# HydrogenSulfate/LFT

Measured on AMD Instinct MI355X. Metric: LF patches/sec (5x5 angRes, 32x32 LR, 4xSR), higher is better.
Workload: dtype bf16; 1 GPU; LFT 5x5 angRes 4xSR inference, batch=4 per GPU, 32x32 LR patches; global_batch=4, parallelism=dp1 (independent shards), streams_per_gpu=1, hip_graph=True, steps_in_flight=2

## Files before the change

### lft_amd/csrc/lft_api.hip

```cpp
#include "../../include/lft_hip.h"
#include "../../include/lft_hip_test.h"
#include <hip/hip_runtime.h>
#include <stdint.h>

#include <cstdarg>
#include <cstdio>
#include <cmath>
#include <map>
#include <mutex>
#include <set>
#include <string>
#include <algorithm>
#include <type_traits>
#include <utility>
#include <vector>

#ifndef LFT_TU
#define LFT_TU 0
#endif

namespace {
#include "lft_kernels_a.cuh"
#include "lft_kernels_b.cuh"
#include "lft_metrics.cuh"
// ... 38 lines not shown
    std::vector<const char*> names;
};
thread_local Profiler g_prof;
inline const char* prof_name(const char* plain, const char* fmt, ...) {
    if (!g_prof.on) return plain;
    static thread_local std::set<std::string> names;
    char buf[96];
    va_list ap;
    va_start(ap, fmt);
    vsnprintf(buf, sizeof(buf), fmt, ap);
    va_end(ap);
    return names.insert(buf).first->c_str();
}
inline void prof_mark(const char* name) {
    if (!g_prof.on) return;
    hipEvent_t e;
    if (hipEventCreate(&e) != hipSuccess) return;
    (void)hipEventRecord(e, g_prof.st);
    g_prof.ev.push_back(e);
    g_prof.names.push_back(name);
}

#define LFT_LAUNCH_OK(name)                                                                  \
    do {                                                                                     \
        hipError_t e_ = hipGetLastError();                                                   \
        if (e_ != hipSuccess) return fail((int)e_, "launch %s: %s", name, hipGetErrorString(e_)); \
        prof_mark(name);                                                                     \
    } while (0)
template <typename Run> int run_profiled(hipStream_t st, int max_records, float* ms_out, const char** names_out, int* n_out, Run&& run) {
    g_prof.on = true; g_prof.st = st; g_prof.ev.clear(); g_prof.names.clear();
    prof_mark("start");
    const int rc = run();
    g_prof.on = false;
    hipError_t e = hipStreamSynchronize(st);
    int n = 0;
    for (size_t i = 1; i < g_prof.ev.size() && n < max_records; ++i, ++n) {
        float ms = 0.0f;
        (void)hipEventElapsedTime(&ms, g_prof.ev[i - 1], g_prof.ev[i]);
        ms_out[n] = ms;
        names_out[n] = g_prof.names[i];
    }
    for (hipEvent_t ev : g_prof.ev) (void)hipEventDestroy(ev);
    g_prof.ev.clear(); g_prof.names.clear();
    *n_out = n;
    if (rc) return rc;
    if (e != hipSuccess) return fail((int)e, "hipStreamSynchronize: %s", hipGetErrorString(e));
    return 0;
}

constexpr int kLayers = 4;

template <auto... Vs, typename V, typename F> int dispatch(V v, F&& f) {
    int rc = 0;
    if (((v == Vs && ((rc = f(std::integral_constant<decltype(Vs), Vs>{})), true)) || ...)) return rc;
    return fail(LFT_ERR_ARG, "internal: no kernel variant for %d", (int)v);
}
template <int V> using int_c = std::integral_constant<int, V>;
template <typename F> int by_prec(int prec, F&& f) {
    if (prec == LFT_PREC_F32) return f(float{});
    if (prec == LFT_PREC_BF16) return f(bf16_t{});
    return f(f16_t{});
}
inline size_t align256(size_t x) { return (x + 255) & ~(size_t)255; }

struct Dims {
    int B, A, V, h, w, hw, s, gp, gt, nchunk;
    long long ntok;
};

int make_dims(int B, int A, int h, int w, int s, int prec, Dims* d) {
    if (prec != LFT_PREC_F32 && prec != LFT_PREC_BF16 && prec != LFT_PREC_F16)
        return fail(LFT_ERR_ARG, "prec must be LFT_PREC_F32, LFT_PREC_BF16 or LFT_PREC_F16, got %d", prec);
    if (B < 1 || A < 1 || h < 1 || w < 1) return fail(LFT_ERR_SHAPE, "B, A, h, w must be positive (B=%d A=%d h=%d w=%d)", B, A, h, w);
    if (s != 2 && s != 4) return fail(LFT_ERR_SHAPE, "scale factor must be 2 or 4, got %d", s);
    if (A * A > 128) return fail(LFT_ERR_UNSUPPORTED, "angRes %d (A*A=%d views > 128) is not implemented in this build", A, A * A);
    if ((long long)B * A * A * h * w > (1LL << 27)) return fail(LFT_ERR_SHAPE, "too many tokens");
    d->B = B; d->A = A; d->V = A * A; d->h = h; d->w = w; d->hw = h * w; d->s = s;
    d->gp = (s + 2) * (s + 2); d->gt = (d->gp + 31) / 32; d->nchunk = 2 * s * s;
    d->ntok = (long long)B * d->V * d->hw;
    return 0;
}

constexpr int kFragsConv = 72, kFragsAng = 64, kFragsSpa1 = 240, kFragsSpa1NoQ = 208, kFragsSpa2 = 176;
inline int frags_up(const Dims& d) { return d.nchunk * (4 + 2 * d.gt); }

struct PackedLayout {
    size_t conv0_w, ln_ang[kLayers], ln_spa[kLayers], ang_pe, petok[kLayers], spa_pe_img;
    size_t w01, s_w01;
    size_t s_conv[3], s_ang[kLayers], s_spa1[kLayers], s_spa2[kLayers], s_up, total;
};

PackedLayout packed_layout(const Dims& d, int prec) {
    const size_t esz = prec == LFT_PREC_F32 ? 4 : 2, fragb = 64 * 8 * esz;
    PackedLayout L;
    size_t o = 0;
    auto take = [&](size_t bytes) { size_t r = o; o = align256(o + bytes); return r; };
    L.conv0_w = take(576 * 4);
    for (int l = 0; l < kLayers; ++l) { L.ln_ang[l] = take(256 * 4); L.ln_spa[l] = take(512 * 4); }
    L.ang_pe = take((size_t)((d.V + 31) / 32) * 2048 * 4);
    for (int l = 0; l < kLayers; ++l) L.petok[l] = take((size_t)((d.hw + 32 * kNwSpa1 - 1) / (32 * kNwSpa1)) * kNwSpa1 * 4096 * esz);
    L.spa_pe_img = take((size_t)d.hw * 64 * esz);
    const bool lp = prec != LFT_PREC_F32;
    L.w01 = take(lp ? 64 * kW01K * 4 : 0);
    L.s_conv[0] = take(kFragsConv * fragb);
    L.s_w01 = take(lp ? kW01Frags * fragb : 0);
    for (int i = 1; i < 3; ++i) L.s_conv[i] = take(kFragsConv * fragb);
    for (int l = 0; l < kLayers; ++l) {
        L.s_ang[l] = take(kFragsAng * fragb);
        L.s_spa1[l] = take(kFragsSpa1 * fragb);
        L.s_spa2[l] = take(kFragsSpa2 * fragb);
    }
    L.s_up = take((size_t)frags_up(d) * fragb);
    L.total = o;
    return L;
}

struct WorkLayout {
    size_t x0, feat, xa, xb, tok, q, k, v, o, g, status, total;
};
WorkLayout work_layout(const Dims& d, int prec) {
    const size_t esz = prec == LFT_PREC_F32 ? 4 : 2;
    WorkLayout W;
    size_t o = 0;
    auto take = [&](size_t bytes) { size_t r = o; o = align256(o + bytes); return r; };
    const size_t n = (size_t)d.ntok;
    W.x0 = take(n * 64 * esz); W.feat = take(n * 64 * esz); W.xa = take(n * 64 * esz); W.xb = take(n * 64 * esz);
    W.tok = take(n * 128 * esz); W.q = take(n * 128 * esz); W.k = take(n * 128 * esz); W.v = take(n * 128 * esz);
    W.o = take(n * 128 * esz);
    W.g = take(n * d.gp * 4);
    W.status = take(256);
    W.total = o;
    return W;
}

template <typename T> size_t lds_conv64(int w) { return WRing<T, kConv64Chunk, kNwConv>::LDS_BYTES + ConvIn<T, kNwConv>::bytes(w) + kNwConv * TileIO<2, T>::BYTES + kConvZeroRow; }
template <typename T> size_t lds_conv64_lr(int w) { return lds_conv64<T>(w) + std::max<size_t>(LrStage<kNwConv>::bytes(w), kConv0WBytes); }
constexpr size_t kLdsParams = 1024;
template <typename T, int CH = kSpaChunk> size_t lds_spa1(int w) {
    return WRing<T, CH, kNwSpa1>::LDS_BYTES + std::max<size_t>(ConvIn<T, kNwSpa1>::bytes(w), (size_t)kNwSpa1 * TileIO<4, T>::BYTES) + kLdsParams + kConvZeroRow;
}
template <typename T> size_t lds_spa2() { return WRing<T, kSpaChunk, kNwSpa2>::LDS_BYTES + kLdsParams + kNwSpa2 * TileIO<4, T>::BYTES; }
template <typename T> size_t lds_up() { return WRing<T, kUpChunk, kNwUp>::LDS_BYTES + kNwUp * TileIO<2, T>::BYTES; }
template <typename T> size_t lds_ang() { return (size_t)kFragsAng * 1024 * FragInfo<T>::PIECES + kLdsParams + 4 * TileIO<2, T>::BYTES; }
constexpr size_t kMaxLds = 160 * 1024;
template <typename K> int allow_lds(K kernel, size_t bytes, const char* name) {
    if (bytes > kMaxLds) return fail(LFT_ERR_SHAPE, "%s needs %zu B of LDS (> 160 KiB): view width too large for this build", name, bytes);
    if (bytes <= 64 * 1024) return 0;
    struct Done { int dev; const void* fn; size_t bytes; };
    static thread_local std::vector<Done> done;
    const void* fn = reinterpret_cast<const void*>(kernel);
    int dev = 0;
    LFT_HIP_OK(hipGetDevice(&dev));
    for (const auto& d : done)
        if (d.dev == dev && d.fn == fn && d.bytes >= bytes) return 0;
    LFT_HIP_OK(hipFuncSetAttribute(fn, hipFuncAttributeMaxDynamicSharedMemorySize, (int)bytes));
    done.push_back(Done{dev, fn, bytes});
    return 0;
}

template <typename P> P* at(const void* base, size_t off) { return reinterpret_cast<P*>(const_cast<char*>(static_cast<const char*>(base)) + off); }
inline unsigned blocks_for(long long items, int per_block) { return (unsigned)((items + per_block - 1) / per_block); }

PackOp lin_op(const float* src, int row0, int nrows, int ld, int k0, int ksteps, int kmap, float scale, int kmul = 1, int kadd = 0) {
    PackOp p{};
    p.src = src; p.kind = 0; p.row0 = row0; p.nrows = nrows; p.ntiles = (nrows + 31) / 32; p.ld = ld;
    p.kmul = kmul; p.kadd = kadd; p.k0 = k0; p.ksteps = ksteps; p.kmap = kmap; p.scale = scale; p.s = 0; p.frag0 = 0;
    return p;
}
void conv_ops(std::vector<PackOp>& v, const float* w, int nout) {
    for (int tap = 0; tap < 9; ++tap)
        for (int ks = 0; ks < 4; ++ks) v.push_back(lin_op(w, 0, nout, 576, 16 * ks, 1, 0, 1.0f, 9, tap));
}

template <typename T>
int run_pack(std::vector<PackOp>& ops, T* dst, int expect_frags, hipStream_t st) {
    int total = 0;
    size_t i = 0;
    while (i < ops.size()) {
        PackArgs a{};
        int nf = 0;
        while (i < ops.size() && a.nops < LFT_PACK_MAXOPS) {
            a.op[a.nops] = ops[i];
            a.op[a.nops].frag0 = nf;
            nf += ops[i].ntiles * ops[i].ksteps;
            ++a.nops; ++i;
        }
        k_pack<T><<<nf, 64, 0, st>>>(a, dst + (size_t)total * 512);
        LFT_LAUNCH_OK("k_pack");
        total += nf;
    }
    if (total != expect_frags) return fail(LFT_ERR_ARG, "internal: stream has %d fragments, expected %d", total, expect_frags);
    return 0;
}

template <typename T> bool tok_lane_major(const Dims& d) {
// ... 4 lines not shown
                int nimg, const Dims& d, hipStream_t st, unsigned* status) {
    const size_t l16 = lds_spa1<T, 16>(d.w), l8 = lds_spa1<T, 8>(d.w);
    const size_t share = kMaxLds / kSpaOcc;
    const bool use8 = (l16 > share && l8 <= share) || l16 > kMaxLds;
    const bool lm = !PE_ONLY && tok_lane_major<T>(d);
    return dispatch<8, 16>(use8 ? 8 : 16, [&](auto CH) {
        return dispatch<true, false>(lm, [&](auto LM) {
            constexpr bool WQ = !(LM && sizeof(T) == 2);
            const size_t lds = CH == 8 ? l8 : l16;
            if (int rc = allow_lds(k_spa1<T, PE_ONLY, CH, LM, WQ>, lds, "k_spa1")) return rc;
            k_spa1<T, PE_ONLY, CH, LM, WQ><<<nwg, 64 * kNwSpa1, lds, st>>>(in, ws, ln, petok, tok, q, k, v, pe_out, nimg, d.h, d.w, status);
            return 0;
        });
    });
}

template <typename T>
int pack_impl(const float* const* P, void* packed, const Dims& d, int prec, hipStream_t st) {
    const PackedLayout L = packed_layout(d, prec);
    const float kAngScale = 0.35355339059327373f * LFT_LOG2E;
    const float kSpaScale = 0.25f * LFT_LOG2E;
    int rc;
    k_copy_f32<<<3, 256, 0, st>>>(P[0], at<float>(packed, L.conv0_w), 576);
    LFT_LAUNCH_OK("k_copy_f32");
    for (int i = 0; i < 3; ++i) {
        std::vector<PackOp> ops;
        conv_ops(ops, P[1 + i], 64);
        if ((rc = run_pack<T>(ops, at<T>(packed, L.s_conv[i]), kFragsConv, st))) return rc;
    }
    if constexpr (sizeof(T) == 2) {
        k_compose_w01<<<blocks_for(64 * kW01K, 256), 256, 0, st>>>(P[0], P[1], at<float>(packed, L.w01));
        LFT_LAUNCH_OK("k_compose_w01");
        std::vector<PackOp> ops{lin_op(at<float>(packed, L.w01), 0, 64, kW01K, 0, kW01K / 16, 0, 1.0f)};
        if ((rc = run_pack<ConvLrOp>(ops, at<ConvLrOp>(packed, L.s_w01), kW01Frags, st))) return rc;
    }
    k_pe_tables<T><<<blocks_for(std::max<long long>((long long)((d.V + 31) / 32) * 2048, (long long)d.hw * 64), 256), 256, 0, st>>>(
        at<float>(packed, L.ang_pe), at<T>(packed, L.spa_pe_img), d.V, d.h, d.w);
    LFT_LAUNCH_OK("k_pe_tables");
    for (int l = 0; l < kLayers; ++l) {
        const float* const* q = P + 4 + 18 * l;
        float* lnS = at<float>(packed, L.ln_spa[l]);
        float* lnA = at<float>(packed, L.ln_ang[l]);
        const int srcS[4] = {1, 2, 5, 6}, srcA[4] = {10, 11, 14, 15};
        for (int j = 0; j < 4; ++j) {
            k_copy_f32<<<1, 256, 0, st>>>(q[srcS[j]], lnS + 128 * j, 128);
            k_copy_f32<<<1, 256, 0, st>>>(q[srcA[j]], lnA + 64 * j, 64);
        }
        LFT_LAUNCH_OK("k_copy_f32");
        {
            std::vector<PackOp> ops;
            ops.push_back(lin_op(q[12], 0, 64, 64, 0, 4, 1, kAngScale));
            ops.push_back(lin_op(q[12], 64, 64, 64, 0, 4, 1, 1.0f));
            ops.push_back(lin_op(q[12], 128, 64, 64, 0, 4, 1, 1.0f));
            ops.push_back(lin_op(q[13], 0, 64, 64, 0, 4, 1, 1.0f));
            ops.push_back(lin_op(q[16], 0, 128, 64, 0, 4, 1, 1.0f));
            ops.push_back(lin_op(q[17], 0, 64, 128, 0, 8, 1, 1.0f));
            if ((rc = run_pack<T>(ops, at<T>(packed, L.s_ang[l]), kFragsAng, st))) return rc;
        }
        {
            std::vector<PackOp> ops;
            conv_ops(ops, q[0], 128);
            ops.push_back(lin_op(q[3], 256, 128, 128, 0, 8, 1, 1.0f));
            ops.push_back(lin_op(q[3], 128, 128, 128, 0, 8, 1, 1.0f));
            ops.push_back(lin_op(q[3], 0, 128, 128, 0, 8, 1, kSpaScale));
            if ((rc = run_pack<T>(ops, at<T>(packed, L.s_spa1[l]), kFragsSpa1, st))) return rc;
        }
        {
            std::vector<PackOp> ops;
            ops.push_back(lin_op(q[4], 0, 128, 128, 0, 8, (sizeof(T) == 2 && tok_lane_major<T>(d)) ? 1 : 0, 1.0f));
            for (int c = 0; c < 4; ++c) {
                ops.push_back(lin_op(q[7], 64 * c, 64, 128, 0, 8, 1, 1.0f));
                ops.push_back(lin_op(q[8], 0, 128, 256, 64 * c, 4, 1, 1.0f));
            }
            ops.push_back(lin_op(q[9], 0, 64, 128, 0, 8, 1, 1.0f));
            if ((rc = run_pack<T>(ops, at<T>(packed, L.s_spa2[l]), kFragsSpa2, st))) return rc;
        }
        if ((rc = launch_spa1<T, true>((unsigned)((d.hw + 32 * kNwSpa1 - 1) / (32 * kNwSpa1)), at<T>(packed, L.spa_pe_img), at<T>(packed, L.s_spa1[l]), nullptr, nullptr,
                                       nullptr, nullptr, nullptr, nullptr, at<T>(packed, L.petok[l]), 1, d, st, nullptr))) return rc;
        LFT_LAUNCH_OK("k_spa1<pe>");
    }
    {
        std::vector<PackOp> ops;
        for (int c = 0; c < d.nchunk; ++c) {
            ops.push_back(lin_op(P[76], 32 * c, 32, 64, 0, 4, 1, 1.0f));
            PackOp m = lin_op(P[77], 0, d.gp, 0, 32 * c, 2, 1, 1.0f);
            m.kind = 1; m.s = d.s; m.ntiles = d.gt;
            ops.push_back(m);
        }
        if ((rc = run_pack<T>(ops, at<T>(packed, L.s_up), frags_up(d), st))) return rc;
    }
    return 0;
}

void launch_assemble(const float* lr, const float* g, float* out, int B, int A, int h, int w, int s, hipStream_t st, int gld = 0, unsigned* status = nullptr) {
    const dim3 tg((unsigned)((A * w + 7) / 8) * (unsigned)((A * h + 7) / 8) * (unsigned)B);
    if (!gld) gld = (s + 2) * (s + 2);
    if (s == 2) k_assemble_t<2><<<tg, 256, 0, st>>>(lr, g, out, B, A, h, w, gld, status);
    else k_assemble_t<4><<<tg, 256, 0, st>>>(lr, g, out, B, A, h, w, gld, status);
}

template <typename T>
int init_features_x0(const void* packed, const PackedLayout& L, const float* lr, T* x0, T* ta, T* tb, T* feat, const Dims& d, hipStream_t st) {
    const int nimg = d.B * d.V, nwg = nimg * ((d.hw + 32 * kNwConv - 1) / (32 * kNwConv));
    const size_t lds = lds_conv64<T>(d.w);
    int rc;
    if ((rc = allow_lds(k_conv64<T, 0>, lds, "k_conv64"))) return rc;
    if ((rc = allow_lds(k_conv64<T, 1>, lds, "k_conv64"))) return rc;
    k_conv0<T><<<dim3((unsigned)((d.hw + kConv0Tok - 1) / kConv0Tok), (unsigned)nimg), 256, 0, st>>>(lr, at<float>(packed, L.conv0_w), x0, d.B, d.A, d.h, d.w);
    LFT_LAUNCH_OK("k_conv0");
    k_conv64<T, 0><<<nwg, 64 * kNwConv, lds, st>>>(x0, ta, nullptr, at<T>(packed, L.s_conv[0]), nimg, d.h, d.w, ConvLr{});
    LFT_LAUNCH_OK("k_conv64");
    k_conv64<T, 0><<<nwg, 64 * kNwConv, lds, st>>>(ta, tb, nullptr, at<T>(packed, L.s_conv[1]), nimg, d.h, d.w, ConvLr{});
    LFT_LAUNCH_OK("k_conv64");
    k_conv64<T, 1><<<nwg, 64 * kNwConv, lds, st>>>(tb, feat, x0, at<T>(packed, L.s_conv[2]), nimg, d.h, d.w, ConvLr{});
    LFT_LAUNCH_OK("k_conv64");
    return 0;
}
template <typename T>
int init_features(const void* packed, const PackedLayout& L, const float* lr, T* x0, T* ta, T* tb, T* feat, const Dims& d, hipStream_t st) {
    if constexpr (sizeof(T) == 4) return init_features_x0<T>(packed, L, lr, x0, ta, tb, feat, d, st);
    else {
        const int nimg = d.B * d.V, nwg = nimg * ((d.hw + 32 * kNwConv - 1) / (32 * kNwConv));
        const size_t lds = lds_conv64_lr<T>(d.w);
        int rc;
        if (L.s_w01 + kW01Frags * 1024 != L.s_conv[1]) return fail(LFT_ERR_ARG, "internal: W01 fragments are not in front of conv_init.2's stream");
        if ((rc = allow_lds(k_conv64_lr<T>, lds, "k_conv64"))) return rc;
        if ((rc = allow_lds(k_conv64<T, 2>, lds, "k_conv64"))) return rc;
        k_conv64_lr<T><<<nwg, 64 * kNwConv, lds, st>>>(lr, tb, at<T>(packed, L.s_w01), d.A, nimg, d.h, d.w);
        LFT_LAUNCH_OK("k_conv64");
        k_conv64<T, 2><<<nwg, 64 * kNwConv, lds, st>>>(tb, feat, nullptr, at<T>(packed, L.s_conv[2]), nimg, d.h, d.w,
                                                      ConvLr{lr, at<float>(packed, L.conv0_w), d.A});
        LFT_LAUNCH_OK("k_conv64");
        return 0;
    }
}
template <typename T, int CT, int LL>
int ang_multi(const void* packed, const PackedLayout& L, int l, const T* in, T* out, const Dims& d, hipStream_t st, unsigned* status) {
    constexpr bool WLDS = sizeof(T) == 2;
    constexpr int NG = (sizeof(T) == 2 && CT <= 3) ? 2 : 1;
    constexpr size_t FB = 1024 * FragInfo<T>::PIECES;
    const size_t lds = (WLDS ? 64 * FB : 0) + 1024 + (size_t)NG * CT * 8 * FB + (size_t)NG * CT * TileIO<2, T>::BYTES;
    const int npix = d.B * d.hw;
    int rc;
    const unsigned grid = std::min<unsigned>(blocks_for(npix, NG), 256u * (unsigned)std::max<size_t>(1, kMaxLds / lds));
    if ((rc = allow_lds(k_ang_multi<T, CT, WLDS, NG, LL>, lds, "k_ang_multi"))) return rc;
    k_ang_multi<T, CT, WLDS, NG, LL><<<grid, 64 * CT * NG, lds, st>>>(in, out, at<T>(packed, L.s_ang[l]), at<float>(packed, L.ln_ang[l]),
                                                                     at<float>(packed, L.ang_pe), d.V, d.hw, npix, status);
    LFT_LAUNCH_OK("k_ang");
    return 0;
}
template <typename T>
int ang_block(const void* packed, const PackedLayout& L, int l, const T* in, T* out, const Dims& d, hipStream_t st, unsigned* status = nullptr) {
    auto multi = [&](auto CT, auto LL) { return ang_multi<T, CT, LL>(packed, L, l, in, out, d, st, status); };
    if (d.V > 100) return multi(int_c<4>{}, int_c<13>{});
    if (d.V > 96) return multi(int_c<4>{}, int_c<9>{});
    if (d.V > 64) return multi(int_c<3>{}, int_c<9>{});
    if (d.V == 64) return multi(int_c<2>{}, int_c<16>{});
    if (d.V > 32) return multi(int_c<2>{}, int_c<9>{});
    const int npix = d.B * d.hw;
    const size_t lds = lds_ang<T>();
    int rc;
    const unsigned grid = std::min<unsigned>(blocks_for(npix, 4), 256u * (unsigned)std::max<size_t>(1, kMaxLds / lds));
    if ((rc = allow_lds(k_ang<T, 13>, lds, "k_ang"))) return rc;
    k_ang<T, 13><<<grid, 256, lds, st>>>(in, out, at<T>(packed, L.s_ang[l]), at<float>(packed, L.ln_ang[l]),
                                         at<float>(packed, L.ang_pe), d.V, d.hw, npix, status);
    LFT_LAUNCH_OK("k_ang");
    return 0;
}
template <typename T>
int spa_part_a(const void* packed, const PackedLayout& L, int l, const T* in, void* ws, const WorkLayout& W, const Dims& d, hipStream_t st) {
    const int nimg = d.B * d.V, nwg = nimg * ((d.hw + 32 * kNwSpa1 - 1) / (32 * kNwSpa1));
    int rc;
// ... 866 lines not shown
```

### lft_amd/csrc/lft_common.cuh

```cuda
#pragma once
#include <hip/hip_runtime.h>
#include <stdint.h>
#include <utility>

typedef __bf16 bf16_t;
typedef float f32x2 __attribute__((ext_vector_type(2)));
__device__ __forceinline__ f32x2 p2_fma(f32x2 a, f32x2 b, f32x2 c) { return __builtin_elementwise_fma(a, b, c); }
typedef float f32x4 __attribute__((ext_vector_type(4)));
typedef float f32x16 __attribute__((ext_vector_type(16)));
typedef __bf16 bf16x4 __attribute__((ext_vector_type(4)));
typedef __bf16 bf16x8 __attribute__((ext_vector_type(8)));
typedef _Float16 f16_t;
typedef _Float16 f16x4 __attribute__((ext_vector_type(4)));
typedef _Float16 f16x8 __attribute__((ext_vector_type(8)));
template <typename T> struct H16;
template <> struct H16<bf16_t> { typedef bf16x4 v4; typedef bf16x8 v8; };
template <> struct H16<f16_t> { typedef f16x4 v4; typedef f16x8 v8; };
typedef unsigned int raw16 __attribute__((ext_vector_type(4), may_alias));

#define LFT_DEV static __device__ __forceinline__
#define LFT_MEM __device__ __forceinline__

#ifdef LFT_EXPERIMENT
#include "lft_experiment.cuh"
// ... 79 lines not shown
}
template <typename T> LFT_DEV Frag<T> load_wfrag(const T* __restrict__ stream, int f, int lane) {
    return frag_from_pieces(reinterpret_cast<const char*>(stream) + (size_t)f * 1024 * FragInfo<T>::PIECES, lane, T());
}

LFT_DEV void glds_piece(const char* __restrict__ gsrc, char* lds_dst, int lane) {
    __builtin_amdgcn_global_load_lds((const __attribute__((address_space(1))) void*)(gsrc + lane * 16),
                                     (__attribute__((address_space(3))) void*)lds_dst, 16, 0, 0);
}

LFT_DEV void glds16_asm(const char* gsrc_lane, char* lds_dst) {
    unsigned keep;
    const unsigned dst = (unsigned)(size_t)(__attribute__((address_space(3))) char*)lds_dst;
    asm volatile("s_mov_b32 %0, m0\n\ts_mov_b32 m0, %2\n\ts_nop 0\n\tglobal_load_lds_dwordx4 %1, off\n\ts_mov_b32 m0, %0"
                 : "=&s"(keep) : "v"(gsrc_lane), "s"(dst) : "memory");
}

#define LFT_VMCNT_CASE(n) case n: asm volatile("s_waitcnt vmcnt(" #n ")" ::: "memory"); break;
LFT_DEV void wait_vmcnt(int n) {
    switch (n < 0 ? 0 : (n > 63 ? 63 : n)) {
        LFT_VMCNT_CASE(0) LFT_VMCNT_CASE(1) LFT_VMCNT_CASE(2) LFT_VMCNT_CASE(3) LFT_VMCNT_CASE(4) LFT_VMCNT_CASE(5) LFT_VMCNT_CASE(6) LFT_VMCNT_CASE(7)
        LFT_VMCNT_CASE(8) LFT_VMCNT_CASE(9) LFT_VMCNT_CASE(10) LFT_VMCNT_CASE(11) LFT_VMCNT_CASE(12) LFT_VMCNT_CASE(13) LFT_VMCNT_CASE(14) LFT_VMCNT_CASE(15)
        LFT_VMCNT_CASE(16) LFT_VMCNT_CASE(17) LFT_VMCNT_CASE(18) LFT_VMCNT_CASE(19) LFT_VMCNT_CASE(20) LFT_VMCNT_CASE(21) LFT_VMCNT_CASE(22) LFT_VMCNT_CASE(23)
        LFT_VMCNT_CASE(24) LFT_VMCNT_CASE(25) LFT_VMCNT_CASE(26) LFT_VMCNT_CASE(27) LFT_VMCNT_CASE(28) LFT_VMCNT_CASE(29) LFT_VMCNT_CASE(30) LFT_VMCNT_CASE(31)
        LFT_VMCNT_CASE(32) LFT_VMCNT_CASE(33) LFT_VMCNT_CASE(34) LFT_VMCNT_CASE(35) LFT_VMCNT_CASE(36) LFT_VMCNT_CASE(37) LFT_VMCNT_CASE(38) LFT_VMCNT_CASE(39)
        LFT_VMCNT_CASE(40) LFT_VMCNT_CASE(41) LFT_VMCNT_CASE(42) LFT_VMCNT_CASE(43) LFT_VMCNT_CASE(44) LFT_VMCNT_CASE(45) LFT_VMCNT_CASE(46) LFT_VMCNT_CASE(47)
        LFT_VMCNT_CASE(48) LFT_VMCNT_CASE(49) LFT_VMCNT_CASE(50) LFT_VMCNT_CASE(51) LFT_VMCNT_CASE(52) LFT_VMCNT_CASE(53) LFT_VMCNT_CASE(54) LFT_VMCNT_CASE(55)
        LFT_VMCNT_CASE(56) LFT_VMCNT_CASE(57) LFT_VMCNT_CASE(58) LFT_VMCNT_CASE(59) LFT_VMCNT_CASE(60) LFT_VMCNT_CASE(61) LFT_VMCNT_CASE(62) LFT_VMCNT_CASE(63)
    }
}

LFT_DEV void wg_barrier_keep_vm() { asm volatile("s_waitcnt lgkmcnt(0)\n\ts_barrier" ::: "memory"); }
LFT_DEV void wg_barrier_keep_vm_lds_visible() {
    __builtin_amdgcn_s_waitcnt(0xC07F);
    asm volatile("s_barrier" ::: "memory");
}

#define LFT_NOTE_ASM_(kind, ring, slot) asm volatile("; LFT_NOTE " kind " ring=%0 slot=%1" :: "i"(ring), "i"(slot))
#define LFT_DMA_NOTE(kind, ring, slot) do { if (__builtin_constant_p(slot)) LFT_NOTE_ASM_(kind, ring, slot); } while (0)
constexpr int kNoteWRing = 0, kNoteWRingPipe = 1, kNoteKV = 2, kNoteConvIn = 3, kNoteAngW = 4;

template <typename T, int CH, int NW = 4>
struct WRing {
    static constexpr int NBUF = 3;
    static constexpr int FRAG_BYTES = 1024 * FragInfo<T>::PIECES;
    static constexpr int CHUNK_BYTES = CH * FRAG_BYTES;
    static constexpr int LDS_BYTES = NBUF * CHUNK_BYTES;
    static constexpr int PIECES_PER_WAVE = CH * FragInfo<T>::PIECES / NW;
    static_assert((CH * FragInfo<T>::PIECES) % NW == 0, "chunk must split over the workgroup's waves");
    static_assert(PIECES_PER_WAVE <= 12, "counted vmcnt immediates below cover up to 12 pieces per wave");
    const char* g;
    char* lds;
    int lane, wave, pos, nfrag;
    LFT_MEM void init(const T* stream, char* lds_base, int total_frags) {
        g = reinterpret_cast<const char*>(stream); lds = lds_base; nfrag = total_frags; pos = 0;
        lane = threadIdx.x & 63;
        wave = __builtin_amdgcn_readfirstlane(threadIdx.x >> 6);
        issue(0);
        issue(1);
    }
    LFT_MEM void issue(int c) {
        if (c * CH >= nfrag) return;
        const char* src = g + (size_t)c * CHUNK_BYTES;
        char* dst = lds + (c % NBUF) * CHUNK_BYTES;
        const int last = (nfrag - c * CH) * FragInfo<T>::PIECES - 1;
        LFT_DMA_NOTE("DMA", kNoteWRing, c % NBUF);
#pragma unroll
        for (int i = 0; i < PIECES_PER_WAVE; ++i) {
            const int piece = min(wave * PIECES_PER_WAVE + i, last);
            glds_piece(src + piece * 1024, dst + piece * 1024, lane);
        }
    }
    LFT_MEM void wait_landed(bool next_in_flight) { wait_vmcnt(next_in_flight ? PIECES_PER_WAVE : 0); }
    LFT_MEM Frag<T> next() {
        const int c = pos / CH, i = pos % CH;
        if (i == 0) {
            if (c > 0) LFT_DMA_NOTE("DONE", kNoteWRing, (c + NBUF - 1) % NBUF);
            wait_landed((c + 1) * CH < nfrag);
            wg_barrier_keep_vm();
            issue(c + 2);
            LFT_DMA_NOTE("USE", kNoteWRing, c % NBUF);
        }
        ++pos;
        return frag_from_pieces(lds + (c % NBUF) * CHUNK_BYTES + i * FRAG_BYTES, lane, T());
    }
};


template <typename T, int CH, int NW, int NBUF, int NFRAG>
struct WRingPipe {
    static constexpr int FRAG_BYTES = 1024 * FragInfo<T>::PIECES;
    static constexpr int CHUNK_BYTES = CH * FRAG_BYTES;
    static constexpr int LDS_BYTES = NBUF * CHUNK_BYTES;
    static constexpr int PIECES_PER_WAVE = CH * FragInfo<T>::PIECES / NW;
    static constexpr int NCHUNK = (NFRAG + CH - 1) / CH;
    static_assert((CH * FragInfo<T>::PIECES) % NW == 0, "chunk must split over the workgroup's waves");
    static_assert(PIECES_PER_WAVE * (NBUF - 1) <= 63, "counted vmcnt immediate");
    static constexpr int cmin(int a, int b) { return a < b ? a : b; }
    static constexpr int cmax(int a, int b) { return a > b ? a : b; }
    const char* g;
    char* lds;
    int lane, wave, split_slot, split_gap;
    Frag<T> fr0[CH], fr1[CH];
    LFT_MEM void setup(const T* stream, char* lds_base, int split_slot_ = NBUF, int split_gap_ = 0) {
        g = reinterpret_cast<const char*>(stream); lds = lds_base;
        split_slot = split_slot_; split_gap = split_gap_;
        lane = threadIdx.x & 63;
        wave = __builtin_amdgcn_readfirstlane(threadIdx.x >> 6);
    }
    LFT_MEM char* slot(int c) const {
        const int s = c % NBUF;
        return lds + s * CHUNK_BYTES + (s >= split_slot ? split_gap : 0);
    }
    LFT_MEM void issue(int c) {
        if (c * CH >= NFRAG) return;
        const char* src = g + (size_t)c * CHUNK_BYTES;
        char* dst = slot(c);
        const int last = (NFRAG - c * CH) * FragInfo<T>::PIECES - 1;
        LFT_DMA_NOTE("DMA", kNoteWRingPipe, c % NBUF);
#pragma unroll
        for (int i = 0; i < PIECES_PER_WAVE; ++i) {
            const int piece = min(wave * PIECES_PER_WAVE + i, last);
            glds_piece(src + piece * 1024, dst + piece * 1024, lane);
        }
    }
    template <int C> LFT_MEM void fetch() {
        const char* base = slot(C);
        LFT_NOTE_ASM_("USE", kNoteWRingPipe, C % NBUF);
#pragma unroll
        for (int i = 0; i < CH; ++i)
            if (C * CH + i < NFRAG) {
                if constexpr (C & 1) fr1[i] = frag_from_pieces(base + i * FRAG_BYTES, lane, T());
                else fr0[i] = frag_from_pieces(base + i * FRAG_BYTES, lane, T());
            }
        LFT_NOTE_ASM_("DONE", kNoteWRingPipe, C % NBUF);
    }
    LFT_MEM void init(const T* stream, char* lds_base) {
        setup(stream, lds_base);
#pragma unroll
        for (int c = 0; c < NBUF; ++c) issue(c);
    }
    LFT_MEM void start() {
        wait_vmcnt(cmax(0, cmin(NBUF - 1, NCHUNK - 1)) * PIECES_PER_WAVE);
        wg_barrier_keep_vm_lds_visible();
        fetch<0>();
        __builtin_amdgcn_sched_barrier(0);
    }
    template <int POS> LFT_MEM Frag<T> get() {
        constexpr int C = POS / CH, I = POS % CH;
        static_assert(POS >= 0 && POS < NFRAG, "position outside the stream");
        if constexpr (I == 0 && C + 1 < NCHUNK) {
            __builtin_amdgcn_sched_barrier(0);
            wait_vmcnt(cmax(0, cmin(NBUF - 2, NCHUNK - 2 - C)) * PIECES_PER_WAVE);
            wg_barrier_keep_vm_lds_visible();
            issue(C + NBUF);
            fetch<C + 1>();
            __builtin_amdgcn_sched_barrier(0);
        }
        if constexpr (C & 1) return fr1[I];
        else return fr0[I];
    }
};
template <int POS0, int NT_OUT, int KS, typename Ring, typename T, int... I>
LFT_DEV void linear_ring_seq(Ring& ring, const Frag<T> (&x)[KS], f32x16 (&y)[NT_OUT], std::integer_sequence<int, I...>) {
    (mma(ring.template get<POS0 + I>(), x[I % KS], y[I / KS]), ...);
}
// ... 543 lines not shown
```

### lft_amd/csrc/lft_kernels_a.cuh

```cuda
#pragma once
#include "lft_common.cuh"

struct PackOp {
    const float* src;
    int kind, row0, nrows, ntiles, ld, kmul, kadd, k0, ksteps, kmap, frag0, s;
    float scale;
    int order;
};
__host__ __device__ __forceinline__ int wfrag_index(int OT, int KS, int ot, int ks) {
    const int g = ot >> 2, G = OT - 4 * g < 4 ? OT - 4 * g : 4;
    return 4 * g * KS + ks * G + (ot & 3);
}
__host__ __device__ __forceinline__ void wfrag_coords(int OT, int KS, int lf, int order, int& nt, int& ks) {
    if (!order) { nt = lf / KS; ks = lf % KS; return; }
    const int gl = (OT - 1) >> 2, g = lf / (4 * KS) < gl ? lf / (4 * KS) : gl, G = OT - 4 * g < 4 ? OT - 4 * g : 4, rem = lf - 4 * g * KS;
    ks = rem / G; nt = 4 * g + rem % G;
}
constexpr int LFT_PACK_MAXOPS = 40;
struct PackArgs {
    int nops;
    PackOp op[LFT_PACK_MAXOPS];
};

LFT_DEV float upm_entry(const float* __restrict__ w3, int n, int kk, int s) {
    const int I = n / (s + 2) - 1, J = n % (s + 2) - 1;
    const int c = kk / (s * s), i = (kk / s) % s, j = kk % s;
    const int dy = i - I, dx = j - J;
    if (dy < -1 || dy > 1 || dx < -1 || dx > 1) return 0.0f;
    return w3[c * 9 + (dy + 1) * 3 + (dx + 1)];
}

template <typename T>
__global__ __launch_bounds__(64) void k_pack(PackArgs args, T* __restrict__ dst) {
    const int f = blockIdx.x, lane = threadIdx.x, r = lane & 31, h = lane >> 5;
    int oi = 0;
    for (int i = 0; i < args.nops; ++i)
        if (f >= args.op[i].frag0) oi = i;
    const PackOp& op = args.op[oi];
    int nt, ks;
    wfrag_coords(op.ntiles, op.ksteps, f - op.frag0, op.order, nt, ks);
    const int n = 32 * nt + r;
#pragma unroll
    for (int j = 0; j < 8; ++j) {
        const int kk = op.k0 + 16 * ks + (op.kmap ? 8 * (j >> 2) + 4 * h + (j & 3) : 8 * h + j);
        float v = 0.0f;
        if (n < op.nrows) {
            if (op.kind == 0) v = op.scale * op.src[(size_t)(op.row0 + n) * op.ld + kk * op.kmul + op.kadd];
            else if (op.kind == 1) v = upm_entry(op.src, n, kk, op.s);
            else v = kk < (op.s + 2) * (op.s + 2) ? upm_entry(op.src, kk, n, op.s) : 0.0f;
        }
        if constexpr (sizeof(T) == 4) dst[(((size_t)f * 2 + (j >> 2)) * 64 + lane) * 4 + (j & 3)] = (T)v;
        else dst[((size_t)f * 64 + lane) * 8 + j] = (T)v;
    }
}

LFT_DEV float pe_value(int l, int c) {
    const int m = c & 31;
    const float g = (float)pow(10000.0, (double)(2 * m) / 64.0);
    const float p = (float)l / g;
    return (c < 32) ? (float)sin((double)p) : (float)cos((double)p);
}
template <typename T>
__global__ void k_pe_tables(float* __restrict__ ang_pe, T* __restrict__ spa_img, int V, int h, int w) {
    const int idx = blockIdx.x * blockDim.x + threadIdx.x;
    const int ntile = (V + 31) / 32;
    if (idx < ntile * 2048) {
        const int e = idx & 7, lane = (idx >> 3) & 63, k = (idx >> 9) & 3, ct = idx >> 11;
        const int view = ct * 32 + (lane & 31), nt = k >> 1, g = 2 * (k & 1) + (e >> 2);
        const int ch = 32 * nt + 8 * g + 4 * (lane >> 5) + (e & 3);
        ang_pe[idx] = view < V ? pe_value(view, ch) : 0.0f;
    }
    if (idx < h * w * 64) {
        const int p = idx >> 6, c = idx & 63;
        spa_img[idx] = (T)((pe_value(p / w, c) + pe_value(p % w, c)) / 2.0f);
    }
}
__global__ void k_copy_f32(const float* __restrict__ src, float* __restrict__ dst, int n) {
    const int i = blockIdx.x * blockDim.x + threadIdx.x;
    if (i < n) dst[i] = src[i];
}

constexpr int kConv0Tok = 128;
template <typename T>
__global__ __launch_bounds__(256) void k_conv0(const float* __restrict__ lr, const float* __restrict__ w0,
                                               T* __restrict__ out, int B, int A, int h, int w) {
    __shared__ __attribute__((aligned(16))) float wl[8 * 100];
    const int hw = h * w, im = blockIdx.y, V = A * A;
    const int cg = threadIdx.x & 7;
    const int b = im / V, v = im - b * V, a1 = v / A, a2 = v - a1 * A;
    const float* img = lr + (size_t)b * (A * h) * (A * w) + (size_t)(a1 * h) * (A * w) + a2 * w;
    constexpr int NP = kConv0Tok / 32;
    float val[NP][9];
#pragma unroll
    for (int pass = 0; pass < NP; ++pass) {
        const int p = min(blockIdx.x * kConv0Tok + pass * 32 + (int)(threadIdx.x >> 3), hw - 1);
        const int y = p / w, x = p - y * w;
#pragma unroll
        for (int t = 0; t < 9; ++t) {
            const int yy = y + t / 3 - 1, xx = x + t % 3 - 1;
            val[pass][t] = img[min(max(yy, 0), h - 1) * (A * w) + min(max(xx, 0), w - 1)];
        }
    }
    {
        float wv[3];
#pragma unroll
        for (int k = 0; k < 3; ++k) wv[k] = w0[min((int)threadIdx.x + 256 * k, 575)];
#pragma unroll
        for (int k = 0; k < 3; ++k) {
            const int i = (int)threadIdx.x + 256 * k, ch = i / 9, t = i - ch * 9;
            if (i < 576) wl[(ch >> 3) * 100 + (ch & 7) * 12 + t] = wv[k];
        }
    }
    __syncthreads();
#pragma unroll
    for (int pass = 0; pass < NP; ++pass) {
        asm volatile("" : "+v"(val[pass][0]), "+v"(val[pass][1]), "+v"(val[pass][2]), "+v"(val[pass][3]), "+v"(val[pass][4]), "+v"(val[pass][5]),
                          "+v"(val[pass][6]), "+v"(val[pass][7]), "+v"(val[pass][8]));
        const int p = blockIdx.x * kConv0Tok + pass * 32 + (threadIdx.x >> 3);
        if (p >= hw) return;
        const int y = p / w, x = p - y * w;
#pragma unroll
        for (int t = 0; t < 9; ++t) {
            const int yy = y + t / 3 - 1, xx = x + t % 3 - 1;
            val[pass][t] = (yy >= 0 && yy < h && xx >= 0 && xx < w) ? val[pass][t] : 0.0f;
        }
        f32x4 o[2];
#pragma unroll
        for (int c = 0; c < 8; ++c) {
            const f32x4* wq = reinterpret_cast<const f32x4*>(wl + cg * 100 + c * 12);
            const f32x4 w03 = wq[0], w47 = wq[1], w8 = wq[2];
// ... 591 lines not shown
```

### lft_amd/csrc/lft_kernels_b.cuh

```cuda
#pragma once
#include "lft_common.cuh"
#include "lft_kernels_a.cuh"

constexpr int kUpChunk = 8;
constexpr int kSpaChunk = 16;
constexpr int kSpaOcc = 2;
constexpr int kNwSpa1 = 4, kNwSpa2 = 4, kNwUp = 8;
template <typename T, bool PE_ONLY, int CH = kSpaChunk, bool TOKLM = false, bool WITH_Q = true, int NW = kNwSpa1>
__global__ __launch_bounds__(64 * NW, kSpaOcc) void k_spa1(const T* __restrict__ X, const T* __restrict__ ws,
                                              const float* __restrict__ ln, const T* __restrict__ petok,
                                              T* __restrict__ TOK, T* __restrict__ Q, T* __restrict__ K, T* __restrict__ Vv,
                                              T* __restrict__ pe_out, int nimg, int h, int w, unsigned* __restrict__ status) {
    extern __shared__ __attribute__((aligned(16))) char smem[];
    const int lane = threadIdx.x & 63, r = lane & 31, hh = lane >> 5, wave = threadIdx.x >> 6;
    constexpr int TT = 32 * NW;
    const int hw = h * w, tpi = (hw + TT - 1) / TT;
    const int bid = xcd_tile(blockIdx.x, gridDim.x);
    const int im = bid / tpi, p0 = (bid % tpi) * TT;
    const int tl = wave * 32 + r, p = p0 + tl;
    const bool ok = p < hw;
    LFT_STAMP(0);
    typename RawPiece<T>::type pe_raw[16];
    if (!PE_ONLY) load_lane_major_raw<4, T>(petok + (size_t)((p0 >> 5) + wave) * 4096, lane, pe_raw);
    char* lds_in = smem + WRing<T, CH, NW>::LDS_BYTES;
    float* lds_ln = reinterpret_cast<float*>(lds_in + max(ConvIn<T, NW>::bytes(w), NW * TileIO<4, T>::BYTES));
    char* zero_row = reinterpret_cast<char*>(lds_ln) + 1024;
    raw16 lnv = raw16{0u, 0u, 0u, 0u};
    if (!PE_ONLY) lnv = params_load(ln, 256);
    WRing<T, CH, NW> ring;
    ring.init(ws, smem, PE_ONLY ? 144 : (WITH_Q ? 240 : 208));
    stage_conv_input<T, NW>(X + (size_t)im * hw * 64, p0, hw, w, lds_in);
    clear_zero_row(zero_row);
    LFT_STAMP(12);
    wait_staged();
    LFT_STAMP(13);
    if (!PE_ONLY) params_store(lds_ln, 256, lnv);
    __syncthreads();
    LFT_NOTE_ASM_("USE", kNoteConvIn, 0);
    LFT_STAMP(1);
    f32x16 t[4];
    zero_acc<4>(t);
    conv3x3_tile<4, T, NW>(lds_in, zero_row, tl, p / w, p % w, ok, h, w, hh, ring, t);
    LFT_STAMP(2);
    if (PE_ONLY) {
        store_lane_major<4, T>(pe_out + (size_t)((p0 >> 5) + wave) * 4096, lane, t);
        return;
    }
    __syncthreads();
    LFT_STAMP(3);
    const int t0 = p0 + wave * 32, nvalid = max(0, min(32, hw - t0));
    const size_t tile_off = ((size_t)im * hw + min(t0, hw - 1)) * 128;
    char* scr = lds_in + wave * TileIO<4, T>::BYTES;
    if constexpr (TOKLM) store_tile_lm<4, T>(TOK + ((size_t)im * hw + t0) * 128, lane, t);
    else store_tile<4, T>(TOK + tile_off, nvalid, lane, t, scr);
    LFT_STAMP(4);
    Frag<T> nf[8];
    constexpr bool QKVLM = TOKLM && sizeof(T) == 2;
    const size_t lm_off = ((size_t)im * hw + t0) * 128;
    acc_frags<4, T>(t, nf);
#pragma unroll
    for (int half = 0; half < 2; ++half) {
        f32x16 a[2];
        zero_acc<2>(a);
        linear_ring<2, 8, T>(ring, nf, a);
        if constexpr (QKVLM) store_tile_lm<2, T>(Vv + lm_off + half * 2048, lane, a);
        else store_tile<2, T, 128>(Vv + tile_off + 64 * half, nvalid, lane, a, scr);
    }
    LFT_STAMP(6);
    add_acc_raw<4, T>(t, pe_raw, ok);
    unsigned bad = 0;
    layernorm_acc<4, sizeof(T) == 2>(t, lds_ln, lds_ln + 128, hh, bad);
    acc_frags<4, T>(t, nf);
    LFT_STAMP(7);
#pragma unroll
    for (int half = 0; half < 2; ++half) {
        f32x16 a[2];
        zero_acc<2>(a);
        linear_ring<2, 8, T>(ring, nf, a);
        if constexpr (QKVLM) store_tile_lm<2, T>(K + lm_off + half * 2048, lane, a);
        else store_tile<2, T, 128>(K + tile_off + 64 * half, nvalid, lane, a, scr);
    }
    LFT_STAMP(9);
    if constexpr (WITH_Q) {
#pragma unroll
        for (int half = 0; half < 2; ++half) {
            f32x16 a[2];
            zero_acc<2>(a);
// ... 354 lines not shown
        LFT_STAMP(19 + 2 * hg);
        LFT_NOTE_ASM_("DONE", kNoteKV, hg & 1);
        wg_barrier_keep_vm();
        if constexpr (!TOKLM) {
            if (hg < 3) q_load_async(qptr + kQPair * (hg + 1), qptr + kQPair * (hg + 1) + kQHead, qa, qb);
        }
        if (hg < 2) stage(hg + 2, buf);
        else if (hg == 2) {
            LFT_NOTE_ASM_("ALIAS_LT", kNoteWRingPipe, kSpaBSlotsA);
#pragma unroll
            for (int c = 0; c < kSpaBSlotsA; ++c) ring.issue(c);
        } else {
#pragma unroll
            for (int c = kSpaBSlotsA; c < kSpaBSlots; ++c) ring.issue(c);
        }
    }
    char* scr = bufB + kSpaBScratchOfs + wave * TileIO<4, T>::BYTES;
    f32x16 t[4], n[4];
    if constexpr (TOKLM) {
#pragma unroll
        for (int kidx = 0; kidx < 8; ++kidx) {
            const V8 v = __builtin_bit_cast(V8, tokr[kidx]);
#pragma unroll
            for (int j = 0; j < 8; ++j) t[kidx >> 1][8 * (kidx & 1) + j] = (float)v[j];
        }
    } else {
        BlkRows rt = rows; rt.img_row_bytes = w * 256; rt.tok_bytes = 256;
        load_tile_map<4, T>(TOK + tok0 * 128, rt, lane, t, scr);
    }
    LFT_STAMP(26);
    __builtin_amdgcn_s_setprio(0);
    ring.start();
    linear_ring_at<0, 4, 8>(ring, of, t);
    LFT_STAMP(27);
#pragma unroll
    for (int nt = 0; nt < 4; ++nt) n[nt] = t[nt];
    layernorm_acc<4, true>(n, lds_ln, lds_ln + 128, hh, bad);
    Frag<T> f[8];
    acc_frags<4, T>(n, f);
    auto ffn_chunk = [&](auto cc) __attribute__((always_inline)) {
        constexpr int C = decltype(cc)::value;
        f32x16 hid[2];
        zero_acc<2>(hid);
        linear_ring_at<32 + 32 * C, 2, 8>(ring, f, hid);
        Frag<T> hf[4];
        acc_frags_relu<2>(hid, hf);
        linear_ring_at<32 + 32 * C + 16, 4, 4>(ring, hf, t);
    };
    ffn_chunk(std::integral_constant<int, 0>());
    ffn_chunk(std::integral_constant<int, 1>());
    ffn_chunk(std::integral_constant<int, 2>());
    ffn_chunk(std::integral_constant<int, 3>());
    LFT_STAMP(28);
    acc_frags<4, T>(t, f);
    f32x16 y[2];
    zero_acc<2>(y);
    linear_ring_at<160, 2, 8>(ring, f, y);
    LFT_STAMP(29);
    BlkRows ry = rows; ry.img_row_bytes = w * 128; ry.tok_bytes = 128;
    if (SKIP) {
        f32x16 sk[2];
        load_tile_map<2, T>(skip + tok0 * 64, ry, lane, sk, scr);
#pragma unroll
        for (int nt = 0; nt < 2; ++nt) y[nt] += sk[nt];
    }
    if constexpr (YLM) {
        if (qy < h) {
            T* dst = Y + (img0 + (long long)qy * w + x0) * 64 + (32 * hh + bxl + qpx) * 8;
#pragma unroll
            for (int kidx = 0; kidx < 4; ++kidx) {
                V8 v;
#pragma unroll
                for (int j = 0; j < 8; ++j) v[j] = (T)y[kidx >> 1][8 * (kidx & 1) + j];
                store_raw16(reinterpret_cast<char*>(dst + kidx * 512), __builtin_bit_cast(raw16, v));
            }
        }
    } else {
        store_tile_map<2, T>(Y + tok0 * 64, ry, lane, y, scr);
    }
    LFT_STAMP(30);
    publish_status(status, bad);
}

template <typename T, int GT, bool XLM = false, int NW = kNwUp>
__global__ __launch_bounds__(64 * NW) void k_up(const T* __restrict__ X, const T* __restrict__ ws, float* __restrict__ G,
                                            long long ntok, int nchunk, int gp) {
    extern __shared__ __attribute__((aligned(16))) char smem[];
    const int lane = threadIdx.x & 63, r = lane & 31, hh = lane >> 5;
    const long long tok_raw = ((long long)blockIdx.x * NW + (threadIdx.x >> 6)) * 32 + r;
    const bool ok = tok_raw < ntok;
    const long long tok = ok ? tok_raw : ntok - 1;
    const long long t0 = tok_raw - r;
    const int nvalid = (int)max(0LL, min(32LL, ntok - t0));
    char* scr = smem + WRing<T, kUpChunk, NW>::LDS_BYTES + (threadIdx.x >> 6) * TileIO<2, T>::BYTES;
    WRing<T, kUpChunk, NW> ring;
    ring.init(ws, smem, nchunk * (4 + 2 * GT));
    f32x16 x[2];
    if constexpr (XLM) load_tile_lm<2, T>(X + t0 * 64, lane, x);
    else load_tile<2, T>(X + min(t0, ntok - 1) * 64, nvalid, lane, x, scr);
    Frag<T> xf[4];
    acc_frags<2, T>(x, xf);
    f32x16 g[GT];
    zero_acc<GT>(g);
#pragma unroll 2
    for (int c = 0; c < nchunk; ++c) {
        f32x16 u[1];
        zero_acc<1>(u);
        linear_ring<1, 4, T>(ring, xf, u);
#pragma unroll
        for (int i = 0; i < 16; ++i) u[0][i] = lrelu02_fast(u[0][i]);
        Frag<T> uf[2];
        acc_frags<1, T>(u, uf);
        linear_ring<GT, 2, T>(ring, uf, g);
    }
    if (!ok) return;
#pragma unroll
    for (int nt = 0; nt < GT; ++nt)
#pragma unroll
        for (int grp = 0; grp < 4; ++grp) {
            const int base = 32 * nt + 8 * grp + 4 * hh;
            if (base < gp)
                store4(G + tok * gp + base, f32x4{g[nt][4 * grp], g[nt][4 * grp + 1], g[nt][4 * grp + 2], g[nt][4 * grp + 3]});
        }
}

LFT_DEV void cubic_coef(float t, float (&c)[4]) {
    const float A = -0.75f;
    const float x0 = t + 1.0f, x1 = t, x2 = 1.0f - t, x3 = 2.0f - t;
    c[0] = ((A * x0 - 5.0f * A) * x0 + 8.0f * A) * x0 - 4.0f * A;
    c[1] = ((A + 2.0f) * x1 - (A + 3.0f)) * x1 * x1 + 1.0f;
    c[2] = ((A + 2.0f) * x2 - (A + 3.0f)) * x2 * x2 + 1.0f;
    c[3] = ((A * x3 - 5.0f * A) * x3 + 8.0f * A) * x3 - 4.0f * A;
}
LFT_DEV float bicubic_at(const float* __restrict__ view, int stride, int h, int w, int Y, int X, int s) {
    const float sy = ((float)Y + 0.5f) / (float)s - 0.5f, sx = ((float)X + 0.5f) / (float)s - 0.5f;
    const float fy = floorf(sy), fx = floorf(sx);
    float cy[4], cx[4];
    cubic_coef(sy - fy, cy);
    cubic_coef(sx - fx, cx);
    const int iy = (int)fy, ix = (int)fx;
    float acc = 0.0f;
#pragma unroll
    for (int a = 0; a < 4; ++a) {
        const int yy = min(max(iy - 1 + a, 0), h - 1);
        float row = 0.0f;
#pragma unroll
        for (int b = 0; b < 4; ++b) row += cx[b] * view[(size_t)yy * stride + min(max(ix - 1 + b, 0), w - 1)];
        acc += cy[a] * row;
    }
    return acc;
}
__global__ __launch_bounds__(256) void k_bicubic(const float* __restrict__ lr, float* __restrict__ out, int B, int A, int h, int w, int s) {
    const int HR_H = A * h * s, HR_W = A * w * s;
    const int X = blockIdx.x * 256 + threadIdx.x, Y = blockIdx.y, b = blockIdx.z;
    if (X >= HR_W) return;
    const int a1 = Y / (h * s), a2 = X / (w * s);
    const float* view = lr + (size_t)b * (A * h) * (A * w) + (size_t)(a1 * h) * (A * w) + a2 * w;
    out[((size_t)b * HR_H + Y) * HR_W + X] = bicubic_at(view, A * w, h, w, Y - a1 * h * s, X - a2 * w * s, s);
}

template <int S>
__global__ __launch_bounds__(256) void k_assemble_t(const float* __restrict__ lr, const float* __restrict__ G, float* __restrict__ out,
                                                    int B, int A, int h, int w, int gld, unsigned* __restrict__ status) {
    constexpr int TL = 8, HL = TL + 2, GP = (S + 2) * (S + 2), P4 = GP / 4, TS = TL * S;
    __shared__ __attribute__((aligned(16))) float gs[HL * HL * GP];
    const int MH = A * h, MW = A * w, HR_W = MW * S, HR_H = MH * S;
    const int tiles_x = (MW + TL - 1) / TL, tiles_y = (MH + TL - 1) / TL;
    const int bid = xcd_tile(blockIdx.x, gridDim.x);
    const int bx0 = (bid % tiles_x) * TL, by0 = ((bid / tiles_x) % tiles_y) * TL, b = bid / (tiles_x * tiles_y);
    const int hw = h * w, V = A * A;
    const float* Gb = G + (size_t)b * V * hw * gld;
    {
        constexpr int NPC = HL * HL * P4, NIT = (NPC + 255) / 256;
        f32x4 vv[NIT];
#pragma unroll
        for (int i = 0; i < NIT; ++i) {
            const int pidx = min((int)threadIdx.x + 256 * i, NPC - 1);
            const int slot = pidx / P4, part = pidx - slot * P4;
            const int by = min(max(by0 - 1 + slot / HL, 0), MH - 1), bx = min(max(bx0 - 1 + slot % HL, 0), MW - 1);
            const int vy = by / h, py = by - vy * h, vx = bx / w, px = bx - vx * w;
            vv[i] = load4(Gb + ((size_t)(vy * A + vx) * hw + py * w + px) * gld + part * 4);
        }
#pragma unroll
        for (int i = 0; i < NIT; ++i) {
// ... 140 lines not shown
```

Before: 10200 patches/s.

## Restructure bf16 upsample kernel into per-block 16x16 MFMA footprint accumulation

For 16-bit precision, the upsampling stage now repacks its second-stage weights per 2x2 sub-pixel block, so each chunk needs five weight fragments instead of four plus two per output tile. It accumulates small 16x16x32 MFMA tiles and then merges overlapping 6x6 footprints through LDS before storing. The aim is to cut the weight-fragment traffic and the MFMA work in the k_up stage. The cost is added shuffle work (frag_to_blocks), LDS staging and extra fences, and the new host packing kinds must stay consistent with the kernel.

```diff
diff --git a/lft_amd/csrc/lft_api.hip b/lft_amd/csrc/lft_api.hip
--- a/lft_amd/csrc/lft_api.hip
+++ b/lft_amd/csrc/lft_api.hip
@@ -144,7 +144,7 @@
 }
 
 constexpr int kFragsConv = 72, kFragsAng = 64, kFragsSpa1 = 240, kFragsSpa1NoQ = 208, kFragsSpa2 = 176;
-inline int frags_up(const Dims& d) { return d.nchunk * (4 + 2 * d.gt); }
+inline int frags_up(const Dims& d, int prec) { return d.nchunk * (prec == LFT_PREC_F32 ? 4 + 2 * d.gt : kUpBlockFrags); }
 
 struct PackedLayout {
     size_t conv0_w, ln_ang[kLayers], ln_spa[kLayers], ang_pe, petok[kLayers], spa_pe_img;
@@ -172,7 +172,7 @@
         L.s_spa1[l] = take(kFragsSpa1 * fragb);
         L.s_spa2[l] = take(kFragsSpa2 * fragb);
     }
-    L.s_up = take((size_t)frags_up(d) * fragb);
+    L.s_up = take((size_t)frags_up(d, prec) * fragb);
     L.total = o;
     return L;
 }
@@ -343,12 +343,22 @@
     {
         std::vector<PackOp> ops;
         for (int c = 0; c < d.nchunk; ++c) {
-            ops.push_back(lin_op(P[76], 32 * c, 32, 64, 0, 4, 1, 1.0f));
-            PackOp m = lin_op(P[77], 0, d.gp, 0, 32 * c, 2, 1, 1.0f);
-            m.kind = 1; m.s = d.s; m.ntiles = d.gt;
-            ops.push_back(m);
+            if constexpr (sizeof(T) == 2) {
+                const int nb = d.s * d.s / 4;
+                PackOp u = lin_op(P[76], 8 * (c / nb), 32, 64, 0, 4, 1, 1.0f);
+                u.kind = 3; u.s = d.s; u.blk = c % nb;
+                ops.push_back(u);
+                PackOp m = lin_op(P[77], 8 * (c / nb), 32, 0, 0, 1, 0, 1.0f);
+                m.kind = 4; m.s = d.s; m.blk = c % nb;
+                ops.push_back(m);
+            } else {
+                ops.push_back(lin_op(P[76], 32 * c, 32, 64, 0, 4, 1, 1.0f));
+                PackOp m = lin_op(P[77], 0, d.gp, 0, 32 * c, 2, 1, 1.0f);
+                m.kind = 1; m.s = d.s; m.ntiles = d.gt;
+                ops.push_back(m);
+            }
         }
-        if ((rc = run_pack<T>(ops, at<T>(packed, L.s_up), frags_up(d), st))) return rc;
+        if ((rc = run_pack<T>(ops, at<T>(packed, L.s_up), frags_up(d, prec), st))) return rc;
     }
     return 0;
 }
diff --git a/lft_amd/csrc/lft_common.cuh b/lft_amd/csrc/lft_common.cuh
--- a/lft_amd/csrc/lft_common.cuh
+++ b/lft_amd/csrc/lft_common.cuh
@@ -185,6 +185,16 @@
             LFT_DMA_NOTE("USE", kNoteWRing, c % NBUF);
         }
         ++pos;
+        return frag_from_pieces(lds + (c % NBUF) * CHUNK_BYTES + i * FRAG_BYTES, lane, T());
+    }
+    template <int I> LFT_MEM Frag<T> next_at(int c0) {
+        constexpr int i = I % CH;
+        const int c = c0 + I / CH;
+        if constexpr (i == 0) {
+            wait_landed((c + 1) * CH < nfrag);
+            wg_barrier_keep_vm();
+            issue(c + 2);
+        }
         return frag_from_pieces(lds + (c % NBUF) * CHUNK_BYTES + i * FRAG_BYTES, lane, T());
     }
 };
diff --git a/lft_amd/csrc/lft_kernels_a.cuh b/lft_amd/csrc/lft_kernels_a.cuh
--- a/lft_amd/csrc/lft_kernels_a.cuh
+++ b/lft_amd/csrc/lft_kernels_a.cuh
@@ -5,6 +5,7 @@
     const float* src;
     int kind, row0, nrows, ntiles, ld, kmul, kadd, k0, ksteps, kmap, frag0, s;
     float scale;
+    int blk;
     int order;
 };
 __host__ __device__ __forceinline__ int wfrag_index(int OT, int KS, int ot, int ks) {
@@ -28,6 +29,17 @@
     const int dy = i - I, dx = j - J;
     if (dy < -1 || dy > 1 || dx < -1 || dx > 1) return 0.0f;
     return w3[c * 9 + (dy + 1) * 3 + (dx + 1)];
+}
+
+LFT_DEV int up_block_row(int m, int chan0, int blk, int s) {
+    const int i = 2 * (blk >> 1) + ((m >> 1) & 1), j = 2 * (blk & 1) + (m & 1);
+    return (chan0 + (m >> 2)) * s * s + i * s + j;
+}
+LFT_DEV float up_block_entry(const float* __restrict__ w3, int l, int j, int chan0, int blk, int s) {
+    const int p = l & 15, g = l >> 4;
+    const int m = 16 * (j >> 2) + 8 * (g & 1) + 4 * (g >> 1) + (j & 3);
+    const int n = (2 * (blk >> 1) + (p >> 2)) * (s + 2) + 2 * (blk & 1) + (p & 3);
+    return upm_entry(w3, n, up_block_row(m, chan0, blk, s), s);
 }
 
 template <typename T>
@@ -44,8 +56,10 @@
     for (int j = 0; j < 8; ++j) {
         const int kk = op.k0 + 16 * ks + (op.kmap ? 8 * (j >> 2) + 4 * h + (j & 3) : 8 * h + j);
         float v = 0.0f;
-        if (n < op.nrows) {
+        if (op.kind == 4) v = up_block_entry(op.src, lane, j, op.row0, op.blk, op.s);
+        else if (n < op.nrows) {
             if (op.kind == 0) v = op.scale * op.src[(size_t)(op.row0 + n) * op.ld + kk * op.kmul + op.kadd];
+            else if (op.kind == 3) v = op.src[(size_t)up_block_row(n, op.row0, op.blk, op.s) * op.ld + kk];
             else if (op.kind == 1) v = upm_entry(op.src, n, kk, op.s);
             else v = kk < (op.s + 2) * (op.s + 2) ? upm_entry(op.src, kk, n, op.s) : 0.0f;
         }
diff --git a/lft_amd/csrc/lft_kernels_b.cuh b/lft_amd/csrc/lft_kernels_b.cuh
--- a/lft_amd/csrc/lft_kernels_b.cuh
+++ b/lft_amd/csrc/lft_kernels_b.cuh
@@ -3,6 +3,7 @@
 #include "lft_kernels_a.cuh"
 
 constexpr int kUpChunk = 8;
+constexpr int kUpBlockFrags = 5;
 constexpr int kSpaChunk = 16;
 constexpr int kSpaOcc = 2;
 constexpr int kNwSpa1 = 4, kNwSpa2 = 4, kNwUp = 8;
@@ -523,6 +524,13 @@
     publish_status(status, bad);
 }
 
+LFT_DEV void up_row6(const f32x4& a, const f32x4& b, float (&o)[6]) {
+    o[0] = a[0]; o[1] = a[1]; o[2] = a[2] + b[0]; o[3] = a[3] + b[1]; o[4] = b[2]; o[5] = b[3];
+}
+LFT_DEV void lds_store6(float* p, const float (&v)[6]) {
+#pragma unroll
+    for (int k = 0; k < 3; ++k) *reinterpret_cast<f32x2 __attribute__((may_alias))*>(p + 2 * k) = f32x2{v[2 * k], v[2 * k + 1]};
+}
 template <typename T, int GT, bool XLM = false, int NW = kNwUp>
 __global__ __launch_bounds__(64 * NW) void k_up(const T* __restrict__ X, const T* __restrict__ ws, float* __restrict__ G,
                                             long long ntok, int nchunk, int gp) {
@@ -535,12 +543,82 @@
     const int nvalid = (int)max(0LL, min(32LL, ntok - t0));
     char* scr = smem + WRing<T, kUpChunk, NW>::LDS_BYTES + (threadIdx.x >> 6) * TileIO<2, T>::BYTES;
     WRing<T, kUpChunk, NW> ring;
-    ring.init(ws, smem, nchunk * (4 + 2 * GT));
+    ring.init(ws, smem, nchunk * (sizeof(T) == 4 ? 4 + 2 * GT : kUpBlockFrags));
     f32x16 x[2];
     if constexpr (XLM) load_tile_lm<2, T>(X + t0 * 64, lane, x);
     else load_tile<2, T>(X + min(t0, ntok - 1) * 64, nvalid, lane, x, scr);
     Frag<T> xf[4];
     acc_frags<2, T>(x, xf);
+    if constexpr (sizeof(T) == 2) {
+        constexpr int NB = GT == 2 ? 4 : 1;
+        static_assert((8 * kUpBlockFrags) % kUpChunk == 0, "a loop body must be a whole number of ring chunks");
+        f32x4 g[NB][2];
+#pragma unroll
+        for (int b = 0; b < NB; ++b) g[b][0] = g[b][1] = f32x4{0, 0, 0, 0};
+        for (int c8 = 0; c8 < nchunk / 8; ++c8) {
+            const int c0 = c8 * (8 * kUpBlockFrags / kUpChunk);
+            auto chunk = [&](auto qc) {
+                constexpr int Q = decltype(qc)::value, F0 = Q * kUpBlockFrags;
+                f32x16 u[1];
+                zero_acc<1>(u);
+                mma(ring.template next_at<F0>(c0), xf[0], u[0]);
+                mma(ring.template next_at<F0 + 1>(c0), xf[1], u[0]);
+                mma(ring.template next_at<F0 + 2>(c0), xf[2], u[0]);
+                mma(ring.template next_at<F0 + 3>(c0), xf[3], u[0]);
+#pragma unroll
+                for (int i = 0; i < 16; ++i) u[0][i] = lrelu02_fast(u[0][i]);
+                Frag<T> uf[2];
+                acc_frags<1, T>(u, uf);
+                raw16 f0 = __builtin_bit_cast(raw16, uf[0].v), f1 = __builtin_bit_cast(raw16, uf[1].v);
+                frag_to_blocks(f0);
+                frag_to_blocks(f1);
+                const Frag<T> m = ring.template next_at<F0 + 4>(c0);
+                typedef typename H16<T>::v8 V8;
+                g[Q % NB][0] = mfma16k32(m.v, __builtin_bit_cast(V8, raw16{f0[0], f0[1], f1[0], f1[1]}), g[Q % NB][0]);
+                g[Q % NB][1] = mfma16k32(m.v, __builtin_bit_cast(V8, raw16{f0[2], f0[3], f1[2], f1[3]}), g[Q % NB][1]);
+            };
+            chunk(std::integral_constant<int, 0>()); chunk(std::integral_constant<int, 1>());
+            chunk(std::integral_constant<int, 2>()); chunk(std::integral_constant<int, 3>());
+            chunk(std::integral_constant<int, 4>()); chunk(std::integral_constant<int, 5>());
+            chunk(std::integral_constant<int, 6>()); chunk(std::integral_constant<int, 7>());
+        }
+        const int gq = lane >> 4, i16 = lane & 15;
+        if constexpr (NB == 1) {
+#pragma unroll
+            for (int ch = 0; ch < 2; ++ch)
+                if (16 * ch + i16 < nvalid) store4(G + (t0 + 16 * ch + i16) * 16 + 4 * gq, g[0][ch]);
+        } else {
+            static_assert(16 * 36 * 4 <= TileIO<2, T>::BYTES, "a 16-token half of the footprints must fit the tile scratch");
+            float* sf = reinterpret_cast<float*>(scr) + i16 * 36 + gq * 6;
+#pragma unroll
+            for (int ch = 0; ch < 2; ++ch) {
+                float top[6], bot[6];
+                up_row6(g[0][ch], g[1][ch], top);
+                up_row6(g[2][ch], g[3][ch], bot);
+                wave_lds_fence();
+                lds_store6(sf, top);
+                if (gq >= 2) lds_store6(sf + 12, bot);
+                wave_lds_fence();
+                if (gq < 2) {
+#pragma unroll
+                    for (int k = 0; k < 3; ++k) {
+                        const f32x2 t = *reinterpret_cast<const f32x2 __attribute__((may_alias))*>(sf + 12 + 2 * k);
+                        bot[2 * k] += t[0]; bot[2 * k + 1] += t[1];
+                    }
+                    lds_store6(sf + 12, bot);
+                }
+                wave_lds_fence();
+                const int npiece = 9 * max(0, min(16, nvalid - 16 * ch));
+                char* gdst = reinterpret_cast<char*>(G + (t0 + 16 * ch) * 36);
+#pragma unroll
+                for (int k = 0; k < 3; ++k) {
+                    const int idx = 64 * k + lane;
+                    if (idx < npiece) store_raw16(gdst + idx * 16, load_raw16(scr + idx * 16));
+                }
+            }
+        }
+        return;
+    }
     f32x16 g[GT];
     zero_acc<GT>(g);
 #pragma unroll 2
```

Measured after the change: 10240 patches/s, median of 2. About the same (+0.5%).
